# Lindeby/toric-RL-decoder

Measured on AMD Instinct MI355X. Metric: env steps/sec (batched) at d=7 p=0.1, higher is better.
Workload: dtype u64

## Files before the change

### include/toricenv.h

```cpp
#ifndef TORICENV_H
#define TORICENV_H

#include <stdint.h>

#ifdef __cplusplus
extern "C" {
#endif

#define TQ_VERSION 200

#define TQ_OK 0
#define TQ_E_INVALID (-1)
#define TQ_E_HIP (-2)
#define TQ_E_CAPACITY (-3)
#define TQ_E_ACTION (-4)
#define TQ_E_INDEX (-5)
#define TQ_E_RESET (-6)

#define TQ_F32 0
#define TQ_F16 1
#define TQ_BF16 2
#define TQ_U8 3

#define TQ_PERR_FIXED 0
#define TQ_PERR_LINEAR 1
#define TQ_PERR_RANDOM 2

typedef struct tq_env tq_env;

int tq_version(void);
const char* tq_last_error(void);

int tq_create(tq_env** out, int n_envs, int d, int device, uint64_t seed, int64_t first_env_id);
int tq_destroy(tq_env* h);

int tq_set_params(tq_env* h, double p_error_default, double terminal_reward, int max_steps_per_episode);
int tq_set_min_qubit_errors(tq_env* h, int n_errors);
int tq_set_perror_schedule(tq_env* h, int strategy, double p_start, double p_final, double p_delta);

int tq_stack_alloc(int device, uint64_t bytes, void** out);
int tq_stack_free(void* ptr);

int tq_set_xcd_bias(int bias);
int tq_get_xcd_bias(void);
int tq_env_set_xcd_bias(tq_env* h, int bias);
int tq_env_get_xcd_bias(const tq_env* h);

int tq_num_envs(const tq_env* h);
int tq_size(const tq_env* h);

int tq_reset_all(tq_env* h, const double* p_err, void* stream);
int tq_reset_idx(tq_env* h, const int32_t* idx, int n_idx, const double* p_err, void* stream);

int tq_step(tq_env* h, const int32_t* actions, float* rewards, uint8_t* terminals, void* stream);

int tq_get_state(tq_env* h, uint8_t* out, void* stream);
int tq_get_state_idx(tq_env* h, const int32_t* idx, int n_idx, uint8_t* out, void* stream);
int tq_get_qubits(tq_env* h, uint8_t* out, void* stream);
int tq_set_qubits(tq_env* h, const uint8_t* qubits, void* stream);
int tq_get_counters(tq_env* h, uint32_t* episodes, uint32_t* steps, void* stream);
int tq_eval_ground_state(tq_env* h, uint8_t* out, void* stream);
int tq_is_terminal(tq_env* h, uint8_t* out, void* stream);

int tq_persp_count(tq_env* h, int32_t* counts, int64_t* offsets, void* stream);
int tq_persp_write(tq_env* h, const int64_t* offsets, void* out, int32_t* positions,
                   int64_t capacity, int dtype, void* stream);
int tq_persp_write_range(tq_env* h, const int64_t* offsets, int first, int count, void* out,
                         int32_t* positions, int64_t capacity, int dtype, void* stream);

typedef struct tq_event tq_event;
int tq_event_create(tq_event** out, int device);
int tq_event_destroy(tq_event* ev);
int tq_persp_write_signal(tq_env* h, const int64_t* offsets, void* out, int32_t* positions,
                          int64_t capacity, int dtype, tq_event* done, void* stream);
int tq_persp_write_range_signal(tq_env* h, const int64_t* offsets, int first, int count, void* out,
                                int32_t* positions, int64_t capacity, int dtype, tq_event* done, void* stream);
int tq_stream_wait_event(tq_event* ev, void* stream);

int tq_states_reserve(int d, int n_max);
// ... 116 lines not shown
```

### toric-rl-decoder_amd/_lib.py

```python
import ctypes as C
import glob
import os
import subprocess

import numpy as np
import torch

_HERE = os.path.dirname(os.path.abspath(__file__))
LIB_PATH = os.path.join(_HERE, "libtoricenv.so")
CSRC = os.path.join(_HERE, "csrc")

TQ_F32, TQ_F16, TQ_BF16, TQ_U8 = 0, 1, 2, 3
TQ_PERR_FIXED, TQ_PERR_LINEAR, TQ_PERR_RANDOM = 0, 1, 2
TQ_OPT_ADAM, TQ_OPT_RMSPROP = 0, 1
TQ_NET_NN8, TQ_NET_NN17 = 8, 17
TQ_NET_RESNET18, TQ_NET_RESNET34 = 18, 34
TQ_E_INVALID, TQ_E_HIP, TQ_E_CAPACITY, TQ_E_ACTION, TQ_E_INDEX, TQ_E_RESET = -1, -2, -3, -4, -5, -6

_vp, _i, _i64, _u64, _d = C.c_void_p, C.c_int, C.c_int64, C.c_uint64, C.c_double
SYMBOLS = [
    ("tq_version", _i, []),
    ("tq_last_error", C.c_char_p, []),
    ("tq_create", _i, [C.POINTER(_vp), _i, _i, _i, _u64, _i64]),
    ("tq_destroy", _i, [_vp]),
    ("tq_set_params", _i, [_vp, _d, _d, _i]),
    ("tq_set_min_qubit_errors", _i, [_vp, _i]),
    ("tq_set_perror_schedule", _i, [_vp, _i, _d, _d, _d]),
    ("tq_stack_alloc", _i, [_i, _u64, C.POINTER(_vp)]),
    ("tq_stack_free", _i, [_vp]),
    ("tq_set_xcd_bias", _i, [_i]),
    ("tq_get_xcd_bias", _i, []),
    ("tq_env_set_xcd_bias", _i, [_vp, _i]),
    ("tq_env_get_xcd_bias", _i, [_vp]),
    ("tq_num_envs", _i, [_vp]),
    ("tq_size", _i, [_vp]),
    ("tq_reset_all", _i, [_vp, _vp, _vp]),
    ("tq_reset_idx", _i, [_vp, _vp, _i, _vp, _vp]),
    ("tq_step", _i, [_vp, _vp, _vp, _vp, _vp]),
    ("tq_get_state", _i, [_vp, _vp, _vp]),
    ("tq_get_state_idx", _i, [_vp, _vp, _i, _vp, _vp]),
    ("tq_get_qubits", _i, [_vp, _vp, _vp]),
    ("tq_set_qubits", _i, [_vp, _vp, _vp]),
    ("tq_get_counters", _i, [_vp, _vp, _vp, _vp]),
    ("tq_eval_ground_state", _i, [_vp, _vp, _vp]),
    ("tq_is_terminal", _i, [_vp, _vp, _vp]),
    ("tq_persp_count", _i, [_vp, _vp, _vp, _vp]),
    ("tq_persp_write", _i, [_vp, _vp, _vp, _vp, _i64, _i, _vp]),
    ("tq_persp_write_range", _i, [_vp, _vp, _i, _i, _vp, _vp, _i64, _i, _vp]),
    ("tq_event_create", _i, [C.POINTER(_vp), _i]),
    ("tq_event_destroy", _i, [_vp]),
    ("tq_persp_write_signal", _i, [_vp, _vp, _vp, _vp, _i64, _i, _vp, _vp]),
    ("tq_persp_write_range_signal", _i, [_vp, _vp, _i, _i, _vp, _vp, _i64, _i, _vp, _vp]),
    ("tq_stream_wait_event", _i, [_vp, _vp]),
    ("tq_states_reserve", _i, [_i, _i]),
    ("tq_states_persp_count", _i, [_i, _i, _vp, _vp, _vp, _vp]),
    ("tq_states_persp_write", _i, [_i, _i, _vp, _vp, _vp, _vp, _i64, _i, _vp]),
    ("tq_select_action", _i, [_vp, _vp, _vp, _vp, _vp, _vp, _vp, _vp]),
    ("tq_states_select_action", _i, [_i, _vp, _vp, _vp, _vp, _u64, _u64, _i64, _vp, _vp, _vp]),
    ("tq_select_plan", _i, [_vp, _vp, _vp, _vp, _vp, _i64, _vp]),
    ("tq_select_action_planned", _i, [_vp, _vp, _vp, _vp, _vp, _vp, _vp, _vp, _vp]),
    ("tq_states_check", _i, [_vp]),
    ("tq_segment_max", _i, [_vp, _vp, _i, _vp, _vp, _vp]),
    ("tq_td_target", _i, [_vp, _vp, _i, _vp, _vp, C.c_float, C.c_float, C.c_float, _vp, _vp]),
    ("tq_transition_write", _i, [_vp, _vp, _vp, _vp, _vp, _vp]),
    ("tq_states_transition", _i, [_i, _i, _vp, _vp, _vp, _vp, _vp, _vp, _vp]),
    ("tq_transition_block_bytes", _i64, [_i, _i64]),
# ... 150 lines not shown
```

### toric-rl-decoder_amd/csrc/cut_points.hpp

```cpp
#pragma once
#include "lattice.hpp"

namespace tq {

TQ_HD int64_t cut_target(int64_t total, int64_t k, int LG) { return (int64_t)(((uint64_t)total * (uint64_t)k) >> LG); }

TQ_HD int64_t cut_floor(int64_t total, int64_t x, int LG) {
    const int64_t G = (int64_t)1 << LG;
    if (total == 0) return G;
    int64_t k = (int64_t)((double)(x + 1) * (double)G / (double)total);
    k = k < 0 ? 0 : (k > G ? G : k);
    while (k < G && cut_target(total, k + 1, LG) <= x) ++k;
    while (k > 0 && cut_target(total, k, LG) > x) --k;
    return k;
}

constexpr int CUT_NL = 8;
template <class Put>
TQ_HD void cut_thread_entries(const int64_t (&o)[CUT_NL + 1], int64_t i0, int64_t total, int LG, Put&& put) {
    if (o[CUT_NL] <= o[0]) return;
    const int64_t kA = cut_floor(total, o[0], LG) + 1, kB = cut_floor(total, o[CUT_NL], LG);
    for (int64_t k = kA; k <= kB; ++k) {
        const int64_t t = cut_target(total, k, LG);
        int j = 0;
#pragma unroll
        for (int q = 1; q < CUT_NL; ++q) j += o[q] < t;
        put(k, (int32_t)(i0 + j + 1));
    }
}
template <class Put>
TQ_HD void cut_block0_entries(int64_t total, int LG, int tid, int nthreads, Put&& put) {
    const int64_t kz = cut_floor(total, 0, LG);
    for (int64_t k = tid; k <= kz; k += nthreads) put(k, 0);
}

constexpr int CUT_HEADER_WORDS = 3;
TQ_HD constexpr int cut_table_words(int LG) { return (1 << LG) + 1 + CUT_HEADER_WORDS; }
TQ_HD void cut_header_store(int32_t* split, int LG, int64_t total, int64_t N) {
    int32_t* h = split + (1 << LG) + 1;
    h[0] = (int32_t)(uint32_t)total; h[1] = (int32_t)(uint32_t)((uint64_t)total >> 32); h[2] = (int32_t)N;
}
TQ_HD bool cut_header_matches(const int32_t* split, int LG, int64_t p_tab, int64_t e_begin, int64_t e_end) {
    const int32_t* h = split + (1 << LG) + 1;
    const int64_t t_all = (int64_t)(((uint64_t)(uint32_t)h[1] << 32) | (uint32_t)h[0]);
    return t_all == p_tab && e_begin == 0 && (int64_t)h[2] == e_end;
}

}
```

### toric-rl-decoder_amd/csrc/stream_range.hpp

```cpp
#pragma once
#include "cut_points.hpp"

namespace tq {

TQ_HD void slot_fine_parts(int large, int idx, int RR, int bias, int& f_lo, int& f_hi) {
    f_lo = idx * 2 * RR + (large ? 0 : RR + bias);
    f_hi = f_lo + (large ? RR + bias : RR - bias);
}

struct StreamRange {
    int64_t org, porg;
    uint32_t head, a0, a1;
    uint32_t phead, pa0, pa1;
    int64_t need_extra;
    bool last, has_stack, has_pos;
};
TQ_HD StreamRange stream_range(int64_t Q0, int64_t Q1, int64_t p_all, int NQ, int esize, bool want_pos) {
    StreamRange r;
    const int LE = 128 / esize;
    r.last = Q1 >= p_all;
    const int64_t S0 = Q0 * NQ, S1 = Q1 * NQ;
    r.org = S0 / LE * LE;
    r.head = (uint32_t)(S0 - r.org);  r.a0 = r.head ? (uint32_t)LE : 0u;
    int64_t A1 = (S1 + LE - 1) / LE * LE;
    if (r.last || A1 > p_all * NQ) A1 = p_all * NQ;
    r.a1 = A1 > r.org ? (uint32_t)(A1 - r.org) : 0u;
    r.porg = Q0 * 3 / 32 * 32;
    r.phead = (uint32_t)(Q0 * 3 - r.porg);  r.pa0 = r.phead ? 32u : 0u;
    int64_t PA1 = (Q1 * 3 + 31) / 32 * 32;
    if (r.last || PA1 > p_all * 3) PA1 = p_all * 3;
    r.pa1 = PA1 > r.porg ? (uint32_t)(PA1 - r.porg) : 0u;
    const int64_t ne_s = (A1 - S1 + NQ - 1) / NQ, ne_p = (PA1 - Q1 * 3 + 2) / 3;
    r.need_extra = r.last ? 0 : ((want_pos && ne_p > ne_s) ? ne_p : ne_s);
    r.has_stack = r.a1 > r.a0;  r.has_pos = want_pos && r.pa1 > r.pa0;
    return r;
}

}
```

### toric-rl-decoder_amd/csrc/stream_write.hpp

```cpp
#pragma once
#include "kernels.hpp"
#include "stream_range.hpp"

namespace tq {

constexpr int ERR_INTERNAL = 32;
constexpr int STREAM_SLOT_WORDS = 4;
constexpr int STREAM_SPIN_LIMIT = 1 << 21;

__device__ __forceinline__ uint32_t lds_peek(const uint32_t& w) {
    return (uint32_t)__builtin_amdgcn_readfirstlane((int)__hip_atomic_load(&w, __ATOMIC_RELAXED, __HIP_MEMORY_SCOPE_WORKGROUP));
}
__device__ __forceinline__ void lds_after_peek() { __builtin_amdgcn_fence(__ATOMIC_ACQUIRE, "wavefront"); }
__device__ __forceinline__ void lds_publish(uint32_t& w, uint32_t v, int lane) {
    __builtin_amdgcn_fence(__ATOMIC_RELEASE, "wavefront");
    if (lane == 0) __hip_atomic_store(&w, v, __ATOMIC_RELAXED, __HIP_MEMORY_SCOPE_WORKGROUP);
}
__device__ __forceinline__ uint64_t readlane64(uint64_t x, int l) {
    const uint32_t lo = (uint32_t)__builtin_amdgcn_readlane((int)(uint32_t)x, l);
    const uint32_t hi = (uint32_t)__builtin_amdgcn_readlane((int)(uint32_t)(x >> 32), l);
    return ((uint64_t)hi << 32) | lo;
}
template <int CNT>
__device__ __forceinline__ uint32_t lds_min(const uint32_t* w, int lane) {
    uint32_t c = 0xFFFFFFFFu;
    if (lane < CNT) c = __hip_atomic_load(&w[lane], __ATOMIC_RELAXED, __HIP_MEMORY_SCOPE_WORKGROUP);
#pragma unroll
    for (int o = 1; o < CNT; o <<= 1) { const uint32_t t = (uint32_t)__shfl_xor((int)c, o, 64); c = t < c ? t : c; }
    return (uint32_t)__builtin_amdgcn_readfirstlane((int)c);
}

template <int D, class OrFn>
__device__ __forceinline__ void emit_at(uint32_t pos, const typename Lat<D>::B& ov, const typename Lat<D>::B& op, OrFn&& orfn) {
    using S = PStream<D>;
    const uint32_t base = pos >> 5;
    const int sh = (int)(pos & 31);
    uint32_t prev = 0;
#pragma unroll
    for (int j = 0; j <= S::ND; ++j) {
        const uint32_t cur = j < S::ND ? S::string_dword(ov, op, j) : 0u;
// ... 92 lines not shown
    __device__ __forceinline__ void range_known() { t_first = since() & 0xFFFFull; }
    __device__ __forceinline__ void lattice_loaded() { if (!n_items) t_first |= (since() & 0xFFFFull) << 16; ++n_items; }
    __device__ __forceinline__ void lattice_in_ring() { if (n_items == 1 && !(t_first >> 32)) t_first |= (since() & 0xFFFFull) << 32; }
    __device__ __forceinline__ void out(unsigned long long* stats, int waves, int wave) const {
        unsigned long long* o = stats + ((size_t)blockIdx.x * waves + wave) * 4;
        o[0] = now() - t_begin; o[1] = t_wait;
        o[2] = (t_rt << 32) | (__builtin_amdgcn_s_memrealtime() & 0xFFFFFFFFull); o[3] = (n_items & 0xFFFFull) | (t_first << 16);
    }
};
__device__ __forceinline__ void give_up(uint32_t& abort, int* err, int lane) {
    if (lane == 0) { __hip_atomic_store(&abort, 1u, __ATOMIC_RELAXED, __HIP_MEMORY_SCOPE_WORKGROUP); atomicOr(err, ERR_INTERNAL); }
}
template <int SLEEP, class Stats, class Pred>
__device__ __forceinline__ bool wait_until(uint32_t& abort, int* err, int lane, Stats& st, Pred&& pred) {
    const unsigned long long t0 = st.now();
    for (int spin = 0; spin < STREAM_SPIN_LIMIT; ++spin) {
        if (pred()) { lds_after_peek(); st.waited(t0); return true; }
        if (lds_peek(abort)) return false;
        __builtin_amdgcn_s_sleep(SLEEP);
    }
    give_up(abort, err, lane);
    return false;
}
template <int NP>
__device__ __forceinline__ uint32_t produced(const uint32_t* pq, int lane) {
    uint32_t v = 0xFFFFFFFFu;
    if (lane < NP) v = __hip_atomic_load(&pq[lane], __ATOMIC_RELAXED, __HIP_MEMORY_SCOPE_WORKGROUP);
    uint32_t m = 0xFFFFFFFFu;
#pragma unroll
    for (int l = 0; l < NP; ++l) { const uint32_t x = (uint32_t)__builtin_amdgcn_readlane((int)v, l); m = x < m ? x : m; }
    return m;
}

template <class K>
__device__ __forceinline__ bool stream_setup(StreamCtx<typename K::Out>& c, typename K::Lds& S, int64_t capacity,
                                             int64_t e_begin, int64_t e_end, const int32_t* __restrict__ split, int lg, int bias,
                                             unsigned int* __restrict__ slots, int wave, int lane) {
    using L = typename K::L;
    const int RR = (1 << lg) / (int)gridDim.x;
    const int64_t p_tab = c.offsets[e_end] - c.offsets[e_begin];
    if (!slots || bias >= RR || p_tab * (int64_t)(K::NQ * sizeof(typename K::Out)) < (int64_t)(64 << 20)) bias = 0;
    const bool take = bias > 0;
    __shared__ int slot_s[2];
    if (threadIdx.x == 0) {
        int large = !(blockIdx.x & 1), idx = (int)(blockIdx.x >> 1);
        if (take) {
            unsigned xcc;
            asm volatile("s_getreg_b32 %0, hwreg(HW_REG_XCC_ID)" : "=s"(xcc));
            large = !(xcc & 1u);
            const unsigned half = gridDim.x >> 1;
            unsigned t = atomicAdd(&slots[large], 1u);
            if (t >= half) { large ^= 1; t = atomicAdd(&slots[large], 1u); }
            idx = t < half ? (int)t : -1;
        }
        slot_s[0] = large; slot_s[1] = idx;
    }
    for (uint32_t i = threadIdx.x; i < (K::BMASK + 1u) / 4; i += blockDim.x) reinterpret_cast<uint4*>(S.bits)[i] = make_uint4(0u, 0u, 0u, 0u);
    if (threadIdx.x == 0) S.abort = 0u;
    if (threadIdx.x < K::NP) S.pq[threadIdx.x] = 0u;
    if (threadIdx.x < K::NPW) S.pcons[threadIdx.x] = 0u;
    if (threadIdx.x < K::NS) S.cons[threadIdx.x] = 0u;
    __syncthreads();
    if (threadIdx.x == 64 * K::NS && take) {
        __threadfence();
        if (atomicAdd(&slots[2], 1u) == gridDim.x - 1u) { slots[0] = 0u; slots[1] = 0u; __threadfence(); slots[2] = 0u; }
    }
    if (slot_s[1] < 0) {
        if (threadIdx.x == 0) atomicOr(c.err, ERR_INTERNAL);
        return false;
    }
    int f_lo, f_hi;
    slot_fine_parts(slot_s[0], slot_s[1], RR, bias, f_lo, f_hi);
    const bool by_tab = split && cut_header_matches(split, lg, p_tab, e_begin, e_end);
    int64_t e_lo, e_hi;
    if (by_tab) {
        e_lo = split[f_lo]; e_hi = split[f_hi];
    } else {
        __shared__ int64_t cut[2];
        if (wave < 2) {
            const int64_t e = find_cut(c.offsets, e_begin, e_end, wave ? f_hi : f_lo, lg, lane);
            if (lane == 0) cut[wave] = e;
        }
        __syncthreads();
        e_lo = cut[0]; e_hi = cut[1];
    }
    e_lo = e_lo < e_begin ? e_begin : (e_lo > e_end ? e_end : e_lo);
    e_hi = e_hi < e_lo ? e_lo : (e_hi > e_end ? e_end : e_hi);
    const int64_t off0 = c.offsets[e_begin];
    int64_t p_all = c.offsets[e_end] - off0;
    int64_t e_stop = e_end;
    if (p_all > capacity) {
        if (blockIdx.x == 0 && threadIdx.x == 0) atomicOr(c.err, ERR_CAPACITY);
        int64_t lo = e_begin, hi = e_end;
        while (lo < hi) {
            const int64_t mid = (lo + hi + 1) >> 1;
            if (c.offsets[mid] - off0 <= capacity) lo = mid; else hi = mid - 1;
        }
        e_stop = lo;
        p_all = c.offsets[e_stop] - off0;
        e_lo = e_lo < e_stop ? e_lo : e_stop;
        e_hi = e_hi < e_stop ? e_hi : e_stop;
    }
    const int64_t Q0 = c.offsets[e_lo] - off0, Q1 = c.offsets[e_hi] - off0;
    if (Q0 < 0 || Q1 < Q0 || Q1 > p_all) {
        if (threadIdx.x == 0) atomicOr(c.err, ERR_INTERNAL);
        return false;
    }
    if (p_all == 0 && e_stop == e_end) {
        for (int64_t e = e_begin + (int64_t)blockIdx.x * blockDim.x + threadIdx.x; e < e_end; e += (int64_t)gridDim.x * blockDim.x) {
            typename L::B v, pl;
#pragma unroll
            for (int k = 0; k < L::W; ++k) { v.w[k] = c.vp[(int64_t)k * c.N + e]; pl.w[k] = c.vp[((int64_t)L::W + k) * c.N + e]; }
            if (L::persp_count(v, pl) != 0) atomicOr(c.err, ERR_INTERNAL);
        }
        return false;
    }
    c.r = stream_range(Q0, Q1, p_all, K::NQ, (int)sizeof(typename K::Out), c.pos != nullptr);
    c.off0 = off0; c.e_lo = e_lo; c.e_stop = e_stop; c.Q0 = Q0; c.QT = Q1 + c.r.need_extra;
    return c.r.has_stack || c.r.has_pos;
}

template <class K, class Stats>
__device__ __forceinline__ bool storer_wave(const StreamCtx<typename K::Out>& c, typename K::Lds& S, int s, int lane, Stats& st) {
    using OutT = typename K::Out;  using Enc = OutEnc<OutT>;
    constexpr int NS = K::NS, CPW = K::CPW, VEC = K::VEC, EPC = K::EPC;
    const uint32_t head = c.r.head, a0 = c.r.a0, a1 = c.r.a1;
    if (!c.r.has_stack) return false;
    __builtin_amdgcn_s_setprio(3);
    constexpr int U = CPW < 4 ? CPW : 4;
    static_assert(CPW % U == 0, "window must be a whole number of trips");
    const uint32_t nchunks = (a1 - a0 + EPC - 1) / EPC;
    const uint32_t lane_el = (uint32_t)lane * VEC;
    const int sh = (int)((a0 + lane_el) & 31u);
    const bool zero_lane = (lane % K::LPD) == 0;
    char* __restrict__ obase = reinterpret_cast<char*>(c.out + c.r.org);
    uint32_t prod_c = 0;
// ... 101 lines not shown
    for (int t = lane; t < 4 * D; t += 64) {
        const int sel = t / D, k = t - sel * D;
        B src;
#pragma unroll
        for (int w = 0; w < W; ++w) src.w[w] = sel == 0 ? v.w[w] : (sel == 1 ? pl.w[w] : (sel == 2 ? rv.w[w] : rp.w[w]));
        const B r = (src.shl(k * D) | src.shr(DD - k * D)) & L::full();
#pragma unroll
        for (int w = 0; w < W; ++w) T.rr[sel][k][w] = r.w[w];
    }
    for (int c = lane; c < K::NQ; c += 64) {
        const int l = c >= DD, bit = c - l * DD;
        if (l ? e1.get(bit) : e0.get(bit)) {
            const int row = bit / D, col = bit - row * D;
            const int k = l ? n0 + e1.rank(bit) : e0.rank(bit);
            const uint32_t hp = (uint32_t)l | ((uint32_t)row << 8) | ((uint32_t)col << 16);
            T.hpos[k] = hp;
            if (has_pos) posr[(q0 + (uint32_t)k) & K::PMASK] = hp;
        }
    }
}
template <class K>
__device__ __forceinline__ void emit_hit(const ProdTables<K::D>& PT, uint32_t* bits, bool has_stack, int k, uint32_t pos) {
    using PS = PStream<K::D>;
    typename K::L::B a, c, low;
    const uint32_t hp = PT.t.hpos[k];
    const int layer = (int)(hp & 255u), i = (int)((hp >> 8) & 255u), jj = (int)(hp >> 16);
    int rs, cs;
    PS::hit_shifts(layer, i, jj, rs, cs);
#pragma unroll
    for (int w = 0; w < K::L::W; ++w) { a.w[w] = PT.t.rr[2 * layer][rs][w]; c.w[w] = PT.t.rr[2 * layer + 1][rs][w]; low.w[w] = PT.low[cs][w]; }
    const auto ov = PS::roll_cols_masked(a, cs, low), op = PS::roll_cols_masked(c, cs, low);
    if (has_stack) emit_at<K::D>(pos, ov, op, [&](uint32_t idx, uint32_t val) { atomicOr(&bits[idx & K::BMASK], val); });
}
template <class K, class Stats>
__device__ __forceinline__ bool producer_wave(const StreamCtx<typename K::Out>& c, typename K::Lds& S, int p, int lane, Stats& st) {
    using L = typename K::L;  using B = typename L::B;
    constexpr int W = L::W, NP = K::NP, NQ = K::NQ;
    const bool has_stack = c.r.has_stack, has_pos = c.r.has_pos;
    const uint32_t head = c.r.head;
    st.range_known();
    ProdTables<K::D>& PT = S.tab[p];
    if (lane < K::D) {
        const B m = L::lowcols(lane);
#pragma unroll
        for (int w = 0; w < W; ++w) PT.low[lane][w] = m.w[w];
    }
    uint32_t lw_c = c.r.a0, pc_c = 0u;
    auto wait_room = [&](uint32_t bits_end, uint32_t q_end) __attribute__((always_inline)) -> bool {
        auto fits = [&]() {
            return (lw_c == 0xFFFFFFFFu || bits_end + 64u <= lw_c + K::RING_BITS) && (!has_pos || pc_c == 0xFFFFFFFFu || q_end <= pc_c + K::RP);
        };
        return fits() || wait_until<8>(S.abort, c.err, lane, st, [&] {
            lw_c = has_stack ? lds_min<K::NS>(S.cons, lane) : 0xFFFFFFFFu;
            if (has_pos) pc_c = lds_min<K::NPW>(S.pcons, lane);
            return fits();
        });
    };
    for (int64_t Lb = 0;; Lb += 64 * NP) {
        const int64_t e_l = c.e_lo + Lb + (int64_t)lane * NP + p;
        const bool in = e_l < c.e_stop;
        uint64_t vv[W], pp[W];
#pragma unroll
        for (int k = 0; k < W; ++k) {
            vv[k] = in ? c.vp[(int64_t)k * c.N + e_l] : 0ull;
            pp[k] = in ? c.vp[((int64_t)W + k) * c.N + e_l] : 0ull;
        }
        const int64_t oo = in ? c.offsets[e_l] - c.off0 : (int64_t)0x7fffffffffffffffll;
        const int64_t oo1 = in ? c.offsets[e_l + 1] - c.off0 : (int64_t)0x7fffffffffffffffll;
        const uint64_t inmask = __ballot(in && oo < c.QT);
        if (!inmask) break;
        const int cnt = __popcll(inmask);
        for (int j = 0; j < cnt; ++j) {
            B v, pl, e0, e1;
#pragma unroll
            for (int k = 0; k < W; ++k) { v.w[k] = readlane64(vv[k], j); pl.w[k] = readlane64(pp[k], j); }
            L::hit_masks(v, pl, e0, e1);
            const int n0 = e0.popc();
            const int n = n0 + e1.popc();
            if (readlane64((uint64_t)oo1, j) - readlane64((uint64_t)oo, j) != (uint64_t)n) { give_up(S.abort, c.err, lane); return false; }
            if (n == 0) continue;
            const uint32_t q0 = (uint32_t)((int64_t)readlane64((uint64_t)oo, j) - c.Q0);
            const uint32_t bit0 = head + q0 * (uint32_t)NQ;
            st.lattice_loaded();
            lds_publish(S.pq[p], q0, lane);
            const uint32_t pass1 = (uint32_t)((K::WHOLE || n < 64) ? n : 64);
            if (!wait_room(bit0 + pass1 * (uint32_t)NQ, q0 + (uint32_t)n)) return false;
            build_tables<K>(PT.t, S.posr, has_pos, v, pl, e0, e1, n0, q0, lane);
            wave_lds_sync();
            for (int kb = 0; kb < n; kb += 64) {
                if (!K::WHOLE && kb) {
                    lds_publish(S.pq[p], q0 + (uint32_t)kb, lane);
                    const uint32_t upto = (uint32_t)(n < kb + 64 ? n : kb + 64);
                    if (!wait_room(bit0 + upto * (uint32_t)NQ, q0 + (uint32_t)n)) return false;
                }
                const int k = kb + lane;
                if (k >= n) continue;
                emit_hit<K>(PT, S.bits, has_stack, k, head + (q0 + (uint32_t)k) * (uint32_t)NQ);
            }
            wave_lds_sync();
            st.lattice_in_ring();
        }
        if (cnt < 64) break;
    }
    lds_publish(S.pq[p], 0xFFFFFFFFu, lane);
    return true;
}

template <int D, typename OutT, int NS, int NP, int CPW, int RB_LOG, int RP_LOG, bool STATS = false, int NPW = 1>
__global__ __launch_bounds__(64 * (NS + NPW + NP)) void k_persp_stream(
        const uint64_t* __restrict__ vp, int64_t N, const int64_t* __restrict__ offsets, OutT* __restrict__ out, int32_t* __restrict__ pos,
        int64_t capacity, int* __restrict__ err, int64_t e_begin, int64_t e_end, const int32_t* __restrict__ split, int lg, int bias,
        unsigned int* __restrict__ slots, unsigned long long* __restrict__ stats = nullptr) {
    using K = StreamShape<D, OutT, NS, NP, CPW, RB_LOG, RP_LOG, NPW>;
    StreamStats<STATS> st;
    __shared__ typename K::Lds S;
    const int wave = __builtin_amdgcn_readfirstlane(threadIdx.x >> 6), lane = threadIdx.x & 63;
    StreamCtx<OutT> c{vp, N, offsets, out, pos, err};
    if (!stream_setup<K>(c, S, capacity, e_begin, e_end, split, lg, bias, slots, wave, lane)) return;
    const bool done = wave >= NS + NPW ? producer_wave<K>(c, S, wave - NS - NPW, lane, st)
                    : wave < NS        ? storer_wave<K>(c, S, wave, lane, st)
                                       : positions_wave<K>(c, S, wave - NS, lane, st);
    if (done && lane == 0) st.out(stats, NS + NPW + NP, wave);
}

}
```

### toric-rl-decoder_amd/csrc/toricenv.hip

```cpp
#include <stdlib.h>
#include <atomic>
#include <string.h>

#include <mutex>
#include <new>

#include "abi_util.hpp"
#include "stream_write.hpp"
#include "select_kernels.hpp"
#include "replay.hpp"

namespace {

struct DeviceCtx {
    std::mutex mu;
    uint16_t* lut[tq::N_SIZES] = {};
    int* err = nullptr;
    void* ws = nullptr;
    size_t ws_bytes = 0;
    int num_cus = 0;
};
constexpr int SPLIT_MAX = 256;
constexpr int SPLIT_LG = 13;
constexpr int N_SLOT_SETS = 8;
constexpr int XCD_BIAS_DEFAULT = 5;
static std::atomic<int> g_xcd_bias{-1};
static int xcd_bias() {
    int b = g_xcd_bias.load(std::memory_order_relaxed);
    if (b < 0) {
        b = XCD_BIAS_DEFAULT;
        if (const char* e = getenv("TORICENV_XCD_BIAS"); e && *e) { const int v = atoi(e); b = v < 0 ? 0 : (v > 16 ? 16 : v); }
        g_xcd_bias.store(b, std::memory_order_relaxed);
    }
    return b;
}
DeviceCtx g_ctx[MAX_DEVICES];

int decode_latch(int flag) {
    if (flag & tq::ERR_ACTION) return fail(TQ_E_ACTION, "an action outside the lattice or with op not in 1..3 was applied");
    if (flag & tq::ERR_CAPACITY) return fail(TQ_E_CAPACITY, "perspective stack capacity exceeded");
    if (flag & tq::ERR_INTERNAL)
        return fail(TQ_E_INVALID, "stack write refused: the offsets are not the scan of these lattices' perspective counts "
                                  "(stale, shifted or from another batch), or a wave gave up waiting; or a planned selection "
                                  "whose plan was made with another eps or before a step");
    if (flag & tq::ERR_INDEX) return fail(TQ_E_INDEX, "tq_reset_idx: an index outside [0, n_envs) was given");
    if (flag & tq::ERR_RESET_DUP) return fail(TQ_E_INDEX, "tq_reset_idx: an index was listed more than once");
    if (flag & tq::ERR_RESET_ROUNDS)
        return fail(TQ_E_RESET, "a reset drew %d rounds without producing a defect (p_error too small)", tq::MAX_RESET_ROUNDS);
    return TQ_OK;
}

int get_lut(int dev, int d, hipStream_t stream, const uint16_t** out) {
    DeviceCtx& c = g_ctx[dev];
    std::lock_guard<std::mutex> lock(c.mu);
    const int slot = tq::size_slot(d);
    if (!c.lut[slot]) {
        const int nq = 2 * d * d;
        const size_t bytes = (2 * (size_t)nq * nq + 15) & ~(size_t)15;
        uint16_t* p = nullptr;
        HIPCHECK(hipMalloc(&p, bytes));
        HIPCHECK(hipMemsetAsync(p, 0, bytes, stream));
        if (int rc = by_size(d, [&](auto D) { return launch_1d(tq::k_build_lut<D()>, (int64_t)nq * nq, stream, p); })) return rc;
        HIPCHECK(hipStreamSynchronize(stream));
        c.lut[slot] = p;
    }
    if (!c.err) {
        HIPCHECK(hipMalloc((void**)&c.err, sizeof(int)));
        HIPCHECK(hipMemset(c.err, 0, sizeof(int)));
// ... 4 lines not shown
        c.num_cus = prop.multiProcessorCount;
    }
    *out = c.lut[slot];
    return TQ_OK;
}

int launch_scan(const int32_t* counts, int64_t* partial, bool partial_valid, int64_t* offsets, int32_t* counts_out,
                int64_t n, hipStream_t stream, int32_t* split) {
    const unsigned blocks = (unsigned)((n + tq::SCAN_CHUNK - 1) / tq::SCAN_CHUNK);
    if (!partial_valid)
        hipLaunchKernelGGL(tq::k_scan_partials, grid1(n), dim3(BLOCK_1D), 0, stream, counts, partial, n);
    hipLaunchKernelGGL(tq::k_scan_final, dim3(blocks), dim3(256), 0, stream, counts, partial, offsets, counts_out, n, split,
                       SPLIT_LG);
    KCHECK();
    return TQ_OK;
}

template <int D, int ES>
struct StreamCfg {
    static constexpr int NS = D <= 5 ? (D == 5 && ES == 2 ? 3 : 2) : 4;
    static constexpr int NPW = (ES < 4 && D >= 5) ? 2 : 1;
    static constexpr int NP = D >= 17 ? 3 : (D >= 13 ? 8 - NPW : 16 - NS - NPW);
    static constexpr int CPW = 8, RB = 14, RP = 12;
};
template <int D, typename OutT>
int launch_persp_write_t(const uint64_t* vp, int64_t n, const int64_t* offsets, void* out, int32_t* pos,
                         int64_t capacity, int* err, hipStream_t stream, int64_t first, int64_t count,
                         const int32_t* split, unsigned int* slots, int bias, hipEvent_t done) {
    using C = StreamCfg<D, (int)sizeof(OutT)>;
    if ((double)count * (2.0 * D * D) * (2.0 * D * D) / SPLIT_MAX * 1.5 > 2.0e9)
        return fail(TQ_E_INVALID, "lattice range too large for one stack write (%lld lattices of d=%d)", (long long)count, D);
    return launch_signal(tq::k_persp_stream<D, OutT, C::NS, C::NP, C::CPW, C::RB, C::RP, false, C::NPW>, dim3(SPLIT_MAX),
                         dim3(64 * (C::NS + C::NPW + C::NP)), stream, done, vp, n, offsets, out, pos, capacity, err, first,
                         first + count, split, SPLIT_LG, (D >= 7 && sizeof(OutT) >= 2) ? bias : 0, slots, nullptr);
}

template <int D>
int launch_persp_write(const uint64_t* vp, int64_t n, const int64_t* offsets, void* out, int32_t* pos,
                       int64_t capacity, int dtype, int* err, hipStream_t stream, int64_t first, int64_t count,
                       const int32_t* split, unsigned int* slots = nullptr, int bias = 0, hipEvent_t done = nullptr) {
    if (count == 0) {
        if (done) HIPCHECK(hipEventRecord(done, stream));
        return TQ_OK;
    }
    switch (dtype) {
        case TQ_F32: return launch_persp_write_t<D, float>(vp, n, offsets, out, pos, capacity, err, stream, first, count, split, slots, bias, done);
        case TQ_F16: return launch_persp_write_t<D, __half>(vp, n, offsets, out, pos, capacity, err, stream, first, count, split, slots, bias, done);
        case TQ_BF16: return launch_persp_write_t<D, tq::bf16_t>(vp, n, offsets, out, pos, capacity, err, stream, first, count, split, slots, bias, done);
        case TQ_U8: return launch_persp_write_t<D, uint8_t>(vp, n, offsets, out, pos, capacity, err, stream, first, count, split, slots, bias, done);
        default: return fail(TQ_E_INVALID, "unknown dtype %d", dtype);
    }
}

}

struct tq_env {
    int n, d, w, device;
    uint64_t seed;
    int64_t first_env;
    double terminal_reward = 100.0;
    int max_steps = 75;
    int min_err;
    tq::PerrSchedule sched = {TQ_PERR_FIXED, 0.1, 0.1, 0.1, 0.0};
    uint64_t* planes;
    uint64_t* planes_alt;
    uint64_t* prev;
    uint32_t* episodes;
// ... 5 lines not shown
    int* err;
    uint32_t* mark;
    uint32_t reset_epoch;
    void* tblock;
    const uint16_t* lut;
    int num_cus;
    int32_t* split[2];
    const int64_t* split_for[2];
    int split_last;
    unsigned int* slots;
    unsigned write_seq;
    int xcd_bias = -1;
    int32_t* sel_need;
    int64_t* sel_partial;
    DeviceBuffers mem;
};

extern "C" {

int tq_version(void) { return TQ_VERSION; }
int tq_set_xcd_bias(int bias) {
    if (bias < 0 || bias > 16) return fail(TQ_E_INVALID, "xcd bias %d outside 0..16", bias);
    g_xcd_bias.store(bias, std::memory_order_relaxed);
    return TQ_OK;
}
int tq_get_xcd_bias(void) { return xcd_bias(); }
int tq_env_set_xcd_bias(tq_env* h, int bias) {
    if (!h) return fail(TQ_E_INVALID, "NULL handle");
    if (bias < -1 || bias > 16) return fail(TQ_E_INVALID, "xcd bias %d outside -1..16", bias);
    h->xcd_bias = bias;
    return TQ_OK;
}
int tq_env_get_xcd_bias(const tq_env* h) { return !h ? TQ_E_INVALID : (h->xcd_bias >= 0 ? h->xcd_bias : xcd_bias()); }

}

#include "abi_stack_alloc.hpp"

extern "C" {

const char* tq_last_error(void) { return g_err; }

int tq_create(tq_env** out, int n_envs, int d, int device, uint64_t seed, int64_t first_env_id) {
    if (!out) return fail(TQ_E_INVALID, "out is NULL");
    *out = nullptr;
    if (n_envs <= 0) return fail(TQ_E_INVALID, "n_envs must be > 0 (got %d)", n_envs);
    if (!tq::size_ok(d)) return bad_size(d);
    if (first_env_id < 0 || first_env_id + n_envs > 0xFFFFFFFFll)
        return fail(TQ_E_INVALID, "global env ids must fit in 32 bits");
    if (int rc = valid_device(device)) return rc;
    DeviceGuard guard;
    if (int rc = guard.enter_device(device)) return rc;
    tq_env* h = new (std::nothrow) tq_env();
    if (!h) return fail(TQ_E_INVALID, "out of host memory");
    h->n = n_envs; h->d = d; h->w = (d * d + 63) / 64; h->device = device;
    h->seed = seed; h->first_env = first_env_id;
    const size_t N = (size_t)n_envs, W = (size_t)h->w;
    DeviceBuffers& m = h->mem;
    m.zeroed(&h->planes, 6 * W * N * 8);
    m.zeroed(&h->planes_alt, 6 * W * N * 8);
    m.zeroed(&h->prev, 2 * W * N * 8);
    m.zeroed(&h->episodes, N * 4);
    m.zeroed(&h->steps, N * 4);
    m.zeroed(&h->counts, N * 4 + 32);
    m.zeroed(&h->partial, ((N + tq::PART_BLOCK - 1) / tq::PART_BLOCK) * 8);
    m.zeroed(&h->p_roof, N * 8);
    m.zeroed(&h->err, 4);
    m.zeroed(&h->mark, N * 4);
    m.zeroed(&h->tblock, (size_t)tq::block_bytes(h->w, n_envs));
    for (int32_t*& t : h->split) m.zeroed(&t, (size_t)tq::cut_table_words(SPLIT_LG) * sizeof(int32_t));
    m.zeroed(&h->slots, N_SLOT_SETS * tq::STREAM_SLOT_WORDS * sizeof(unsigned int));
    m.zeroed(&h->sel_need, N * 4 + 32);
    m.zeroed(&h->sel_partial, ((N + tq::PART_BLOCK - 1) / tq::PART_BLOCK) * 8);
    if (const hipError_t e = m.err; e != hipSuccess) { tq_destroy(h); return fail(TQ_E_HIP, "hipMalloc failed: %s", hipGetErrorString(e)); }
    if (int rc = get_lut(device, d, nullptr, &h->lut)) { tq_destroy(h); return rc; }
    h->num_cus = g_ctx[device].num_cus;
    if (hipError_t se = hipStreamSynchronize(nullptr); se != hipSuccess) {
        tq_destroy(h);
        return fail(TQ_E_HIP, "hipStreamSynchronize failed: %s", hipGetErrorString(se));
    }
    *out = h;
    return TQ_OK;
}

int tq_destroy(tq_env* h) {
    if (!h) return TQ_OK;
    DeviceGuard guard;
    (void)guard.enter_device(h->device);
    h->mem.release_all();
    delete h;
    return TQ_OK;
}

int tq_set_params(tq_env* h, double p_error_default, double terminal_reward, int max_steps_per_episode) {
    if (!h) return fail(TQ_E_INVALID, "NULL handle");
    const bool p_unused = h->min_err > 0;
    if (!((p_error_default > 0.0 || (p_unused && p_error_default == 0.0)) && p_error_default <= 1.0))
        return fail(TQ_E_INVALID, "p_error must be in (0,1] (0 is accepted only with min_qubit_errors > 0)");
    if (max_steps_per_episode < 1) return fail(TQ_E_INVALID, "max_steps_per_episode must be >= 1");
    h->sched.p_default = p_error_default;
    h->terminal_reward = terminal_reward;
    h->max_steps = max_steps_per_episode;
    return TQ_OK;
}
// ... 154 lines not shown
    (void)hipEventDestroy(ev->ev);
    delete ev;
    return TQ_OK;
}

int tq_stream_wait_event(tq_event* ev, void* stream_) {
    DeviceGuard guard;
    if (int rc = guard.enter(ev)) return rc;
    HIPCHECK(hipStreamWaitEvent((hipStream_t)stream_, ev->ev, 0));
    return TQ_OK;
}

int tq_persp_write_range_signal(tq_env* h, const int64_t* offsets, int first, int count, void* out, int32_t* positions,
                                int64_t capacity, int dtype, tq_event* done, void* stream_) {
    ENTER(h, "handle");
    if (!offsets || !out) return fail(TQ_E_INVALID, "offsets / out is NULL");
    if (capacity < 0) return fail(TQ_E_INVALID, "negative capacity");
    if (first < 0 || count < 0 || (int64_t)first + count > h->n) return fail(TQ_E_INVALID, "lattice range outside [0, n_envs)");
    REQUIRE_ALIGNED16(out, "out");
    REQUIRE_ALIGNED16(positions, "positions");
    if (done) {
        if (done->device != h->device) return fail(TQ_E_INVALID, "the event belongs to device %d, the handle to %d", done->device, h->device);
        hipStreamCaptureStatus cap = hipStreamCaptureStatusNone;
        HIPCHECK(hipStreamIsCapturing(stream, &cap));
        if (cap != hipStreamCaptureStatusNone)
            return fail(TQ_E_INVALID, "tq_persp_write_signal on a capturing stream: capture the plain tq_persp_write");
    }
    const uint64_t* vp = h->planes + (size_t)tq::PL_V * h->w * h->n;
    const int32_t* split = nullptr;
    if (first == 0 && count == h->n) {
        if (offsets == h->split_for[h->split_last]) split = h->split[h->split_last];
        else if (offsets == h->split_for[h->split_last ^ 1]) split = h->split[h->split_last ^ 1];
    }
    unsigned int* slots = h->slots + tq::STREAM_SLOT_WORDS * (h->write_seq++ % N_SLOT_SETS);
    return by_size(h->d, [&](auto D) {
        return launch_persp_write<D()>(vp, h->n, offsets, out, positions, capacity, dtype, h->err, stream, first, count, split,
                                       slots, h->xcd_bias >= 0 ? h->xcd_bias : xcd_bias(), done ? done->ev : nullptr);
    });
}

int tq_persp_write_range(tq_env* h, const int64_t* offsets, int first, int count, void* out, int32_t* positions,
                         int64_t capacity, int dtype, void* stream_) {
    return tq_persp_write_range_signal(h, offsets, first, count, out, positions, capacity, dtype, nullptr, stream_);
}

int tq_persp_write_signal(tq_env* h, const int64_t* offsets, void* out, int32_t* positions, int64_t capacity,
                          int dtype, tq_event* done, void* stream_) {
    if (!h) return fail(TQ_E_INVALID, "NULL handle");
    return tq_persp_write_range_signal(h, offsets, 0, h->n, out, positions, capacity, dtype, done, stream_);
}

int tq_persp_write(tq_env* h, const int64_t* offsets, void* out, int32_t* positions, int64_t capacity,
                   int dtype, void* stream_) {
    if (!h) return fail(TQ_E_INVALID, "NULL handle");
    return tq_persp_write_range_signal(h, offsets, 0, h->n, out, positions, capacity, dtype, nullptr, stream_);
}

static int stateless_enter(int d, hipStream_t stream, int* dev, const uint16_t** lut) {
    if (int rc = current_device(dev)) return rc;
    return get_lut(*dev, d, stream, lut);
}

struct StatesScratch {
    size_t counts_at, partial_at, bytes;
    StatesScratch(int d, int64_t n) {
        const size_t w = (size_t)(d * d + 63) / 64;
        counts_at = 2 * w * (size_t)n * 8;
        partial_at = counts_at + (((size_t)n * 4 + 32 + 15) & ~(size_t)15);
        bytes = partial_at + (((size_t)n + tq::PART_BLOCK - 1) / tq::PART_BLOCK) * 8;
    }
};
// ... 234 lines not shown
```

Before: 228.2 million.

## Replace global slot counters with per-pair claims and overlap cut lookups

The XCD-biased slot assignment in the stream write kernel used three global atomic counters shared by every workgroup, plus a last-block reset. It now uses one padded word per workgroup pair: each pair claims large or small halves with a single atomicAdd, and the second arriver resets the word. Cut-table and offset reads are batched into per-lane loads with readlane, and the three cut points are searched in parallel by separate waves. Producer waves also prefetch their first tile of inputs during setup. The cost is a larger slot buffer and more intricate claim logic. The measured env step metric may not exercise this persp write path much.

After: 231.5 million, median of 6. 1.4% higher.

```diff
diff --git a/include/toricenv.h b/include/toricenv.h
--- a/include/toricenv.h
+++ b/include/toricenv.h
@@ -45,6 +45,8 @@
 int tq_get_xcd_bias(void);
 int tq_env_set_xcd_bias(tq_env* h, int bias);
 int tq_env_get_xcd_bias(const tq_env* h);
+int tq_debug_force_xcc_parity(int parity);
+int tq_debug_slot_words_nonzero(tq_env* h);
 
 int tq_num_envs(const tq_env* h);
 int tq_size(const tq_env* h);
diff --git a/toric-rl-decoder_amd/_lib.py b/toric-rl-decoder_amd/_lib.py
--- a/toric-rl-decoder_amd/_lib.py
+++ b/toric-rl-decoder_amd/_lib.py
@@ -32,6 +32,8 @@
     ("tq_get_xcd_bias", _i, []),
     ("tq_env_set_xcd_bias", _i, [_vp, _i]),
     ("tq_env_get_xcd_bias", _i, [_vp]),
+    ("tq_debug_force_xcc_parity", _i, [_i]),
+    ("tq_debug_slot_words_nonzero", _i, [_vp]),
     ("tq_num_envs", _i, [_vp]),
     ("tq_size", _i, [_vp]),
     ("tq_reset_all", _i, [_vp, _vp, _vp]),
diff --git a/toric-rl-decoder_amd/csrc/cut_points.hpp b/toric-rl-decoder_amd/csrc/cut_points.hpp
--- a/toric-rl-decoder_amd/csrc/cut_points.hpp
+++ b/toric-rl-decoder_amd/csrc/cut_points.hpp
@@ -40,10 +40,14 @@
     int32_t* h = split + (1 << LG) + 1;
     h[0] = (int32_t)(uint32_t)total; h[1] = (int32_t)(uint32_t)((uint64_t)total >> 32); h[2] = (int32_t)N;
 }
+TQ_HD constexpr int cut_header_at(int LG) { return (1 << LG) + 1; }
+TQ_HD bool cut_header_words_match(int32_t h0, int32_t h1, int32_t h2, int64_t p_tab, int64_t e_begin, int64_t e_end) {
+    const int64_t t_all = (int64_t)(((uint64_t)(uint32_t)h1 << 32) | (uint32_t)h0);
+    return t_all == p_tab && e_begin == 0 && (int64_t)h2 == e_end;
+}
 TQ_HD bool cut_header_matches(const int32_t* split, int LG, int64_t p_tab, int64_t e_begin, int64_t e_end) {
-    const int32_t* h = split + (1 << LG) + 1;
-    const int64_t t_all = (int64_t)(((uint64_t)(uint32_t)h[1] << 32) | (uint32_t)h[0]);
-    return t_all == p_tab && e_begin == 0 && (int64_t)h[2] == e_end;
+    const int32_t* h = split + cut_header_at(LG);
+    return cut_header_words_match(h[0], h[1], h[2], p_tab, e_begin, e_end);
 }
 
 }
diff --git a/toric-rl-decoder_amd/csrc/stream_range.hpp b/toric-rl-decoder_amd/csrc/stream_range.hpp
--- a/toric-rl-decoder_amd/csrc/stream_range.hpp
+++ b/toric-rl-decoder_amd/csrc/stream_range.hpp
@@ -6,6 +6,21 @@
 TQ_HD void slot_fine_parts(int large, int idx, int RR, int bias, int& f_lo, int& f_hi) {
     f_lo = idx * 2 * RR + (large ? 0 : RR + bias);
     f_hi = f_lo + (large ? RR + bias : RR - bias);
+}
+
+constexpr int PAIR_WORD_STRIDE = 32;
+TQ_HD constexpr int pair_set_words(int workgroups) { return workgroups / 2 * PAIR_WORD_STRIDE; }
+struct PairClaim {
+    unsigned add;
+    int kind;
+    bool second;
+};
+TQ_HD PairClaim pair_claim(unsigned old, int prefers_large) {
+    PairClaim c;
+    c.add = 1u + 2u * (unsigned)(prefers_large != 0);
+    c.second = old != 0u;
+    c.kind = old == 0u ? (prefers_large != 0) : (old == 1u ? 1 : (old == 3u ? 0 : -1));
+    return c;
 }
 
 struct StreamRange {
diff --git a/toric-rl-decoder_amd/csrc/stream_write.hpp b/toric-rl-decoder_amd/csrc/stream_write.hpp
--- a/toric-rl-decoder_amd/csrc/stream_write.hpp
+++ b/toric-rl-decoder_amd/csrc/stream_write.hpp
@@ -5,7 +5,6 @@
 namespace tq {
 
 constexpr int ERR_INTERNAL = 32;
-constexpr int STREAM_SLOT_WORDS = 4;
 constexpr int STREAM_SPIN_LIMIT = 1 << 21;
 
 __device__ __forceinline__ uint32_t lds_peek(const uint32_t& w) {
@@ -164,62 +163,73 @@
     return m;
 }
 
-template <class K>
+template <class K, class Prefetch>
 __device__ __forceinline__ bool stream_setup(StreamCtx<typename K::Out>& c, typename K::Lds& S, int64_t capacity,
                                              int64_t e_begin, int64_t e_end, const int32_t* __restrict__ split, int lg, int bias,
-                                             unsigned int* __restrict__ slots, int wave, int lane) {
+                                             unsigned int* __restrict__ slots, int force_parity, int wave, int lane, Prefetch&& prefetch) {
     using L = typename K::L;
+    static_assert(K::NS + K::NPW + K::NP >= 4, "waves 1-3 find the pair's cut points");
     const int RR = (1 << lg) / (int)gridDim.x;
-    const int64_t p_tab = c.offsets[e_end] - c.offsets[e_begin];
-    if (!slots || bias >= RR || p_tab * (int64_t)(K::NQ * sizeof(typename K::Out)) < (int64_t)(64 << 20)) bias = 0;
-    const bool take = bias > 0;
-    __shared__ int slot_s[2];
-    if (threadIdx.x == 0) {
-        int large = !(blockIdx.x & 1), idx = (int)(blockIdx.x >> 1);
-        if (take) {
-            unsigned xcc;
-            asm volatile("s_getreg_b32 %0, hwreg(HW_REG_XCC_ID)" : "=s"(xcc));
-            large = !(xcc & 1u);
-            const unsigned half = gridDim.x >> 1;
-            unsigned t = atomicAdd(&slots[large], 1u);
-            if (t >= half) { large ^= 1; t = atomicAdd(&slots[large], 1u); }
-            idx = t < half ? (int)t : -1;
-        }
-        slot_s[0] = large; slot_s[1] = idx;
-    }
-    for (uint32_t i = threadIdx.x; i < (K::BMASK + 1u) / 4; i += blockDim.x) reinterpret_cast<uint4*>(S.bits)[i] = make_uint4(0u, 0u, 0u, 0u);
+    const int pair = (int)(blockIdx.x >> 1);
+    const bool claim = slots && bias > 0 && !(gridDim.x & 1u);
+    int prefers_large = !(blockIdx.x & 1);
+    unsigned old = 0u;
+    if (threadIdx.x == 0 && claim) {
+        unsigned xcc;
+        asm volatile("s_getreg_b32 %0, hwreg(HW_REG_XCC_ID)" : "=s"(xcc));
+        if (force_parity >= 0) xcc = force_parity < 2 ? (unsigned)force_parity : (xcc ^ 1u);
+        prefers_large = !(xcc & 1u);
+        unsigned word = (unsigned)(pair * PAIR_WORD_STRIDE);
+        asm volatile("" : "+v"(word));
+        old = atomicAdd(&slots[word], pair_claim(0u, prefers_large).add);
+    }
+    if (!claim || bias >= RR) bias = 0;
+    int f_lo, f_eq, f_bias, f_hi;
+    slot_fine_parts(1, pair, RR, 0, f_lo, f_eq);
+    slot_fine_parts(0, pair, RR, bias, f_bias, f_hi);
+    const int64_t ow = c.offsets[lane == 1 ? e_end : e_begin];
+    int32_t tw = 0;
+    if (split) {
+        int fi = cut_header_at(lg) + (lane >= 4 && lane < 4 + CUT_HEADER_WORDS ? lane - 4 : 0);
+        fi = lane == 0 ? f_lo : fi;  fi = lane == 1 ? f_eq : fi;  fi = lane == 2 ? f_bias : fi;  fi = lane == 3 ? f_hi : fi;
+        tw = split[fi];
+    }
+    const int64_t off0 = (int64_t)readlane64((uint64_t)ow, 0);
+    int64_t p_all = (int64_t)readlane64((uint64_t)ow, 1) - off0;
+    int64_t cut_lo = __builtin_amdgcn_readlane(tw, 0), cut_eq = __builtin_amdgcn_readlane(tw, 1), cut_bias = __builtin_amdgcn_readlane(tw, 2),
+            cut_hi = __builtin_amdgcn_readlane(tw, 3);
+    const bool by_tab = split && cut_header_words_match(__builtin_amdgcn_readlane(tw, 4), __builtin_amdgcn_readlane(tw, 5),
+                                                        __builtin_amdgcn_readlane(tw, 6), p_all, e_begin, e_end);
+    if (p_all * (int64_t)(K::NQ * sizeof(typename K::Out)) < (int64_t)(64 << 20)) bias = 0;
+    int64_t cut_mid = bias ? cut_bias : cut_eq;
+    __shared__ int64_t cut_s[3];
+    __shared__ int kind_s;
+    if (!by_tab && wave >= 1 && wave <= 3) {
+        const int64_t e = find_cut(c.offsets, e_begin, e_end, wave == 1 ? f_lo : (wave == 2 ? (bias ? f_bias : f_eq) : f_hi), lg, lane);
+        if (lane == 0) cut_s[wave - 1] = e;
+    }
+    constexpr uint32_t THREADS = 64u * (K::NS + K::NPW + K::NP);
+    for (uint32_t i = threadIdx.x; i < (K::BMASK + 1u) / 4; i += THREADS) reinterpret_cast<uint4*>(S.bits)[i] = make_uint4(0u, 0u, 0u, 0u);
     if (threadIdx.x == 0) S.abort = 0u;
     if (threadIdx.x < K::NP) S.pq[threadIdx.x] = 0u;
     if (threadIdx.x < K::NPW) S.pcons[threadIdx.x] = 0u;
     if (threadIdx.x < K::NS) S.cons[threadIdx.x] = 0u;
+    if (threadIdx.x == 0) {
+        const PairClaim pc = pair_claim(old, prefers_large);
+        if (claim && pc.second) __hip_atomic_store(&slots[pair * PAIR_WORD_STRIDE], 0u, __ATOMIC_RELAXED, __HIP_MEMORY_SCOPE_AGENT);
+        kind_s = claim ? pc.kind : prefers_large;
+    }
     __syncthreads();
-    if (threadIdx.x == 64 * K::NS && take) {
-        __threadfence();
-        if (atomicAdd(&slots[2], 1u) == gridDim.x - 1u) { slots[0] = 0u; slots[1] = 0u; __threadfence(); slots[2] = 0u; }
-    }
-    if (slot_s[1] < 0) {
+    int kind = kind_s;
+    if (kind < 0) {
         if (threadIdx.x == 0) atomicOr(c.err, ERR_INTERNAL);
         return false;
     }
-    int f_lo, f_hi;
-    slot_fine_parts(slot_s[0], slot_s[1], RR, bias, f_lo, f_hi);
-    const bool by_tab = split && cut_header_matches(split, lg, p_tab, e_begin, e_end);
-    int64_t e_lo, e_hi;
-    if (by_tab) {
-        e_lo = split[f_lo]; e_hi = split[f_hi];
-    } else {
-        __shared__ int64_t cut[2];
-        if (wave < 2) {
-            const int64_t e = find_cut(c.offsets, e_begin, e_end, wave ? f_hi : f_lo, lg, lane);
-            if (lane == 0) cut[wave] = e;
-        }
-        __syncthreads();
-        e_lo = cut[0]; e_hi = cut[1];
-    }
+    if (!bias) kind = !(blockIdx.x & 1);
+    if (!by_tab) { cut_lo = cut_s[0]; cut_mid = cut_s[1]; cut_hi = cut_s[2]; }
+    int64_t e_lo = kind ? cut_lo : cut_mid, e_hi = kind ? cut_mid : cut_hi;
     e_lo = e_lo < e_begin ? e_begin : (e_lo > e_end ? e_end : e_lo);
     e_hi = e_hi < e_lo ? e_lo : (e_hi > e_end ? e_end : e_hi);
-    const int64_t off0 = c.offsets[e_begin];
-    int64_t p_all = c.offsets[e_end] - off0;
     int64_t e_stop = e_end;
     if (p_all > capacity) {
         if (blockIdx.x == 0 && threadIdx.x == 0) atomicOr(c.err, ERR_CAPACITY);
@@ -233,7 +243,9 @@
         e_lo = e_lo < e_stop ? e_lo : e_stop;
         e_hi = e_hi < e_stop ? e_hi : e_stop;
     }
-    const int64_t Q0 = c.offsets[e_lo] - off0, Q1 = c.offsets[e_hi] - off0;
+    const int64_t qw = c.offsets[lane == 1 ? e_hi : e_lo];
+    prefetch(e_lo, e_stop);
+    const int64_t Q0 = (int64_t)readlane64((uint64_t)qw, 0) - off0, Q1 = (int64_t)readlane64((uint64_t)qw, 1) - off0;
     if (Q0 < 0 || Q1 < Q0 || Q1 > p_all) {
         if (threadIdx.x == 0) atomicOr(c.err, ERR_INTERNAL);
         return false;
@@ -401,8 +413,28 @@
     const auto ov = PS::roll_cols_masked(a, cs, low), op = PS::roll_cols_masked(c, cs, low);
     if (has_stack) emit_at<K::D>(pos, ov, op, [&](uint32_t idx, uint32_t val) { atomicOr(&bits[idx & K::BMASK], val); });
 }
+template <class K>
+struct ProducerLoads {
+    uint64_t vv[K::L::W], pp[K::L::W];
+    int64_t oo, oo1;
+    bool in;
+    __device__ __forceinline__ void load(const uint64_t* __restrict__ vp, int64_t N, const int64_t* __restrict__ offsets, int64_t e_lo,
+                                         int64_t e_stop, int64_t Lb, int p, int lane) {
+        constexpr int W = K::L::W;
+        const int64_t e_l = e_lo + Lb + (int64_t)lane * K::NP + p;
+        in = e_l < e_stop;
+#pragma unroll
+        for (int k = 0; k < W; ++k) {
+            vv[k] = in ? vp[(int64_t)k * N + e_l] : 0ull;
+            pp[k] = in ? vp[((int64_t)W + k) * N + e_l] : 0ull;
+        }
+        oo = in ? offsets[e_l] : 0;
+        oo1 = in ? offsets[e_l + 1] : 0;
+    }
+};
 template <class K, class Stats>
-__device__ __forceinline__ bool producer_wave(const StreamCtx<typename K::Out>& c, typename K::Lds& S, int p, int lane, Stats& st) {
+__device__ __forceinline__ bool producer_wave(const StreamCtx<typename K::Out>& c, typename K::Lds& S, int p, int lane, Stats& st,
+                                              ProducerLoads<K>& ld) {
     using L = typename K::L;  using B = typename L::B;
     constexpr int W = L::W, NP = K::NP, NQ = K::NQ;
     const bool has_stack = c.r.has_stack, has_pos = c.r.has_pos;
@@ -426,16 +458,11 @@
         });
     };
     for (int64_t Lb = 0;; Lb += 64 * NP) {
-        const int64_t e_l = c.e_lo + Lb + (int64_t)lane * NP + p;
-        const bool in = e_l < c.e_stop;
-        uint64_t vv[W], pp[W];
-#pragma unroll
-        for (int k = 0; k < W; ++k) {
-            vv[k] = in ? c.vp[(int64_t)k * c.N + e_l] : 0ull;
-            pp[k] = in ? c.vp[((int64_t)W + k) * c.N + e_l] : 0ull;
-        }
-        const int64_t oo = in ? c.offsets[e_l] - c.off0 : (int64_t)0x7fffffffffffffffll;
-        const int64_t oo1 = in ? c.offsets[e_l + 1] - c.off0 : (int64_t)0x7fffffffffffffffll;
+        if (Lb) ld.load(c.vp, c.N, c.offsets, c.e_lo, c.e_stop, Lb, p, lane);
+        const bool in = ld.in;
+        const uint64_t (&vv)[W] = ld.vv, (&pp)[W] = ld.pp;
+        const int64_t oo = in ? ld.oo - c.off0 : (int64_t)0x7fffffffffffffffll;
+        const int64_t oo1 = in ? ld.oo1 - c.off0 : (int64_t)0x7fffffffffffffffll;
         const uint64_t inmask = __ballot(in && oo < c.QT);
         if (!inmask) break;
         const int cnt = __popcll(inmask);
@@ -479,14 +506,17 @@
 __global__ __launch_bounds__(64 * (NS + NPW + NP)) void k_persp_stream(
         const uint64_t* __restrict__ vp, int64_t N, const int64_t* __restrict__ offsets, OutT* __restrict__ out, int32_t* __restrict__ pos,
         int64_t capacity, int* __restrict__ err, int64_t e_begin, int64_t e_end, const int32_t* __restrict__ split, int lg, int bias,
-        unsigned int* __restrict__ slots, unsigned long long* __restrict__ stats = nullptr) {
+        unsigned int* __restrict__ slots, int force_parity, unsigned long long* __restrict__ stats = nullptr) {
     using K = StreamShape<D, OutT, NS, NP, CPW, RB_LOG, RP_LOG, NPW>;
     StreamStats<STATS> st;
     __shared__ typename K::Lds S;
     const int wave = __builtin_amdgcn_readfirstlane(threadIdx.x >> 6), lane = threadIdx.x & 63;
     StreamCtx<OutT> c{vp, N, offsets, out, pos, err};
-    if (!stream_setup<K>(c, S, capacity, e_begin, e_end, split, lg, bias, slots, wave, lane)) return;
-    const bool done = wave >= NS + NPW ? producer_wave<K>(c, S, wave - NS - NPW, lane, st)
+    ProducerLoads<K> ld;
+    if (!stream_setup<K>(c, S, capacity, e_begin, e_end, split, lg, bias, slots, force_parity, wave, lane, [&](int64_t e_lo, int64_t e_stop) {
+            if (wave >= NS + NPW) ld.load(vp, N, offsets, e_lo, e_stop, 0, wave - NS - NPW, lane);
+        })) return;
+    const bool done = wave >= NS + NPW ? producer_wave<K>(c, S, wave - NS - NPW, lane, st, ld)
                     : wave < NS        ? storer_wave<K>(c, S, wave, lane, st)
                                        : positions_wave<K>(c, S, wave - NS, lane, st);
     if (done && lane == 0) st.out(stats, NS + NPW + NP, wave);
diff --git a/toric-rl-decoder_amd/csrc/toricenv.hip b/toric-rl-decoder_amd/csrc/toricenv.hip
--- a/toric-rl-decoder_amd/csrc/toricenv.hip
+++ b/toric-rl-decoder_amd/csrc/toricenv.hip
@@ -23,6 +23,7 @@
 constexpr int SPLIT_MAX = 256;
 constexpr int SPLIT_LG = 13;
 constexpr int N_SLOT_SETS = 8;
+constexpr int SLOT_SET_WORDS = tq::pair_set_words(SPLIT_MAX);
 constexpr int XCD_BIAS_DEFAULT = 5;
 static std::atomic<int> g_xcd_bias{-1};
 static int xcd_bias() {
@@ -34,6 +35,7 @@
     }
     return b;
 }
+static std::atomic<int> g_force_xcc_parity{-1};
 DeviceCtx g_ctx[MAX_DEVICES];
 
 int decode_latch(int flag) {
@@ -104,7 +106,8 @@
         return fail(TQ_E_INVALID, "lattice range too large for one stack write (%lld lattices of d=%d)", (long long)count, D);
     return launch_signal(tq::k_persp_stream<D, OutT, C::NS, C::NP, C::CPW, C::RB, C::RP, false, C::NPW>, dim3(SPLIT_MAX),
                          dim3(64 * (C::NS + C::NPW + C::NP)), stream, done, vp, n, offsets, out, pos, capacity, err, first,
-                         first + count, split, SPLIT_LG, (D >= 7 && sizeof(OutT) >= 2) ? bias : 0, slots, nullptr);
+                         first + count, split, SPLIT_LG, (D >= 7 && sizeof(OutT) >= 2) ? bias : 0, slots,
+                         g_force_xcc_parity.load(std::memory_order_relaxed), nullptr);
 }
 
 template <int D>
@@ -176,6 +179,11 @@
     return TQ_OK;
 }
 int tq_env_get_xcd_bias(const tq_env* h) { return !h ? TQ_E_INVALID : (h->xcd_bias >= 0 ? h->xcd_bias : xcd_bias()); }
+int tq_debug_force_xcc_parity(int parity) {
+    if (parity < -1 || parity > 2) return fail(TQ_E_INVALID, "xcc parity %d outside -1..2", parity);
+    g_force_xcc_parity.store(parity, std::memory_order_relaxed);
+    return TQ_OK;
+}
 
 }
 
@@ -213,7 +221,7 @@
     m.zeroed(&h->mark, N * 4);
     m.zeroed(&h->tblock, (size_t)tq::block_bytes(h->w, n_envs));
     for (int32_t*& t : h->split) m.zeroed(&t, (size_t)tq::cut_table_words(SPLIT_LG) * sizeof(int32_t));
-    m.zeroed(&h->slots, N_SLOT_SETS * tq::STREAM_SLOT_WORDS * sizeof(unsigned int));
+    m.zeroed(&h->slots, (size_t)N_SLOT_SETS * SLOT_SET_WORDS * sizeof(unsigned int));
     m.zeroed(&h->sel_need, N * 4 + 32);
     m.zeroed(&h->sel_partial, ((N + tq::PART_BLOCK - 1) / tq::PART_BLOCK) * 8);
     if (const hipError_t e = m.err; e != hipSuccess) { tq_destroy(h); return fail(TQ_E_HIP, "hipMalloc failed: %s", hipGetErrorString(e)); }
@@ -434,11 +442,23 @@
         if (offsets == h->split_for[h->split_last]) split = h->split[h->split_last];
         else if (offsets == h->split_for[h->split_last ^ 1]) split = h->split[h->split_last ^ 1];
     }
-    unsigned int* slots = h->slots + tq::STREAM_SLOT_WORDS * (h->write_seq++ % N_SLOT_SETS);
+    unsigned int* slots = h->slots + (size_t)SLOT_SET_WORDS * (h->write_seq++ % N_SLOT_SETS);
     return by_size(h->d, [&](auto D) {
         return launch_persp_write<D()>(vp, h->n, offsets, out, positions, capacity, dtype, h->err, stream, first, count, split,
                                        slots, h->xcd_bias >= 0 ? h->xcd_bias : xcd_bias(), done ? done->ev : nullptr);
     });
+}
+
+int tq_debug_slot_words_nonzero(tq_env* h) {
+    void* stream_ = nullptr;
+    ENTER(h, "handle");
+    (void)stream;
+    HIPCHECK(hipDeviceSynchronize());
+    std::vector<unsigned int> w((size_t)N_SLOT_SETS * SLOT_SET_WORDS);
+    HIPCHECK(hipMemcpy(w.data(), h->slots, w.size() * sizeof(unsigned int), hipMemcpyDeviceToHost));
+    int n = 0;
+    for (unsigned int x : w) n += x != 0u;
+    return n;
 }
 
 int tq_persp_write_range(tq_env* h, const int64_t* offsets, int first, int count, void* out, int32_t* positions,
```
